# lgleznah/mort

Hardware: AMD Instinct MI355X
Metric: Msamples/sec (width x height x spp/s), Scene 1 1200x675 (higher is better)
Workload: dtype f32; 1 GPU; Scene 1 (random-spheres cover) 1200x675, 500 spp nominal = 484 effective, depth 20, megakernel, seed 69420, host LCG scene; mode=mega, partition=rows/8 interleaved over 1 rank(s)

## Files before the change

mort_amd/csrc/hip/dev_math.h:

```cpp
#ifndef MORT_DEV_MATH_H
#define MORT_DEV_MATH_H

#include <hip/hip_runtime.h>
#include <stdint.h>
#include "mort_math.h"

#pragma clang fp contract(off)

#define DEV __host__ __device__ __forceinline__

struct V3 { float x, y, z; };
DEV V3 mk(float x, float y, float z) { V3 r; r.x = x; r.y = y; r.z = z; return r; }
DEV V3 vadd(V3 a, V3 b) { return mk(a.x + b.x, a.y + b.y, a.z + b.z); }
DEV V3 vsub(V3 a, V3 b) { return mk(a.x - b.x, a.y - b.y, a.z - b.z); }
DEV V3 vmul(V3 a, V3 b) { return mk(a.x * b.x, a.y * b.y, a.z * b.z); }
DEV V3 vneg(V3 a) { return mk(-a.x, -a.y, -a.z); }
DEV V3 vscale(float t, V3 v) { return mk(t * v.x, t * v.y, t * v.z); }
DEV V3 vdiv(V3 v, float t) { return vscale(1 / t, v); }
DEV float vdot(V3 u, V3 v) { return u.x * v.x + u.y * v.y + u.z * v.z; }
DEV float vlen2(V3 a) { return a.x * a.x + a.y * a.y + a.z * a.z; }
DEV float vlen(V3 a) { return mort_sqrtf(vlen2(a)); }
DEV V3 vunit(V3 a) { return vdiv(a, vlen(a)); }
DEV V3 vcross(V3 u, V3 v) { return mk(u.y * v.z - u.z * v.y, u.z * v.x - u.x * v.z, u.x * v.y - u.y * v.x); }

// ... 41 lines not shown
        V3 p = mk(a, b, 0);
        if (vlen2(p) < 1) return p;
    }
}
DEV V3 random_cosine_direction(Rng &s) {
    float r1 = random_float(s);
    float r2 = random_float(s);
    float phi = (float)(2 * 3.1415926 * (double)r1);
    float sq = mort_sqrtf(r2);
    float sn, cs;
    mort_sincosf(phi, &sn, &cs);
    float x = cs * sq;
    float y = sn * sq;
    float z = mort_sqrtf(1 - r2);
    return mk(x, y, z);
}
DEV V3 reflect(V3 v, V3 n) { return vsub(v, vscale(2 * vdot(v, n), n)); }
DEV V3 refract(V3 uv, V3 n, float etai_over_etat) {
    double cos_theta = mort_fmin((double)vdot(vneg(uv), n), 1.0);
    V3 r_out_perp = vscale(etai_over_etat, vadd(uv, vscale((float)cos_theta, n)));
    V3 r_out_parallel = vscale((float)(-mort_sqrt(mort_fabs(1.0 - (double)vlen2(r_out_perp)))), n);
    return vadd(r_out_perp, r_out_parallel);
}
DEV float reflectance(float cosine, float ref_idx) {
    float r0 = (1 - ref_idx) / (1 + ref_idx);
    r0 = r0 * r0;
    return r0 + (1 - r0) * mort_powi5f(1 - cosine);
}

struct Onb { V3 u, v, w; };
DEV Onb onb_from_w(V3 w) {
    Onb o;
    V3 unit_w = vunit(w);
    V3 a = ((double)mort_fabsf(unit_w.x) > 0.9) ? mk(0, 1, 0) : mk(1, 0, 0);
    V3 v = vunit(vcross(unit_w, a));
    V3 u = vcross(unit_w, v);
    o.u = u; o.v = v; o.w = unit_w;
    return o;
}
DEV V3 onb_local(const Onb &o, V3 a) { return vadd(vadd(vscale(a.x, o.u), vscale(a.y, o.v)), vscale(a.z, o.w)); }

#endif
```

mort_amd/csrc/hip/dev_scene.h:

```cpp
#ifndef MORT_DEV_SCENE_H
#define MORT_DEV_SCENE_H

#include <stdint.h>
#include "mort_scene.h"

#define DREF(type, idx) (((uint32_t)(type) << 16) | (uint32_t)(idx))
#define DREF_TYPE(r) ((int)((r) >> 16) & 0x7fff)
#define DREF_IDX(r) ((int)((r) & 0xffffu))

struct __attribute__((aligned(16))) DSphere {
    float cx, cy, cz, radius;
    float vx, vy, vz;
    uint32_t mat;
};

struct __attribute__((aligned(16))) DQuad {
    float Q[3], D;
    float u[3], area;
    float v[3]; uint32_t mat;
    float n[3]; uint32_t pad0;
    float w[3]; uint32_t pad1;
};

struct __attribute__((aligned(16))) DBvhNode {
// ... 3 lines not shown
};

struct __attribute__((aligned(16))) DNode2 {
    float x0min, x0max, y0min, y0max;
    float z0min, z0max, x1min, x1max;
    float y1min, y1max, z1min, z1max;
    uint32_t child0, child1;
    float e0, e1;
};
struct __attribute__((aligned(16))) DNode4 {
    float x[3][4], y[3][4], z[3][4], e[4];
    uint32_t child[4];
};
#define MORT_NODE4_X 0
#define MORT_NODE4_Y 3
#define MORT_NODE4_Z 6
#define MORT_NODE4_E 9
#define MORT_NODE4_CHILD 10
struct __attribute__((aligned(16))) DLeaf2 {
    DSphere a, b;
    float xmin, xmax, ymin, ymax, zmin, zmax;
    uint32_t n;
    uint32_t prims;
    uint32_t pad[4];
};
#define MORT_NODE4_PIECES 11
#define MORT_LEAF2_PIECES 7
#define MORT_OWN4_STACK 24
struct __attribute__((aligned(16))) DNodeQ {
    float ox, oy, oz;
    uint32_t exps;
    uint32_t q0;
    uint32_t q1;
    uint32_t q2;
    uint32_t children;
};
#define GLEAF_FIRST(ref) ((ref) & 0x1fffu)
#define GLEAF_COUNT(ref) ((((ref) >> 13) & 3u) + 1u)
#define MORT_OWN_STACK 16
#define MORT_OWN_MAX_DEPTH 15
#ifndef MORT_GEN_LEAF_MAX
#define MORT_GEN_LEAF_MAX 2
#endif
#define GENT(kind, chain, idx) (((uint32_t)(kind) << 31) | ((uint32_t)(chain) << 24) | (uint32_t)(idx))
#define GENT_QUAD(e) ((e) >> 31)
#define GENT_CHAIN(e) (((e) >> 24) & 0x7fu)
#define GENT_IDX(e) ((e) & 0xffffffu)

enum { XF_TRANSLATE = 0, XF_ROTATE_Y = 1 };
struct __attribute__((aligned(16))) DXform {
    int kind;
    float a, b, c;
};

enum { ITEM_BVH = 0, ITEM_SPHERES = 1, ITEM_QUADS = 2, ITEM_MEDIUM = 3 };
struct __attribute__((aligned(16))) DItem {
    int kind;
    int first, count;
    int chain_first, chain_count;
    uint32_t mat;
    int medium;
    int pad0;
};

struct __attribute__((aligned(16))) DLambert { float r, g, b; uint32_t tex; };
struct __attribute__((aligned(16))) DMetal { float r, g, b, fuzz; };
struct __attribute__((aligned(8))) DDielectric { float ior, inv_ior; };
struct __attribute__((aligned(16))) DSolid { float r, g, b, pad; };
struct __attribute__((aligned(16))) DChecker { float inv_scale; uint32_t even, odd; uint32_t pad; };
struct __attribute__((aligned(16))) DImage { uint32_t offset; int width, height, pad; };

enum { LIGHT_NONE = -1, LIGHT_INVALID = 0, LIGHT_SPHERE = 1, LIGHT_QUAD = 2, LIGHT_LIST = 3 };

struct DScene {
    const DItem *items;     int n_items;
    const DItem *subitems;  int n_subitems;
    const DBvhNode *nodes;  int n_nodes;
    const DSphere *spheres; int n_spheres;
    const DQuad *quads;     int n_quads;
    const DXform *xforms;   int n_xforms;
    const double *neg_inv_density; int n_media;
    const DLambert *lambert; const DMetal *metal; const DDielectric *dielectric;
    const DLambert *dlight;  const DLambert *isotropic;
    const DSolid *solid; const DChecker *checker; const DImage *image;
    const DImage *image_hbm;
    const unsigned char *texels;
    const float *noise;
    const DSphere *wspheres; const DQuad *wquads;
    const int *list_types; const int *list_idxs;
    const int *list_first; const int *list_count;
// ... 6 lines not shown
```

mort_amd/csrc/hip/mega_bvh.h:

```cpp
#ifndef MORT_MEGA_BVH_H
#define MORT_MEGA_BVH_H

#include "dev_render.h"


struct FastArgs {
    RenderArgs r;
    const unsigned char *hot_src;
    uint32_t hot_bytes;
    uint32_t off_nodes4, off_leafrecs, off_lambert, off_metal, off_diel, off_dlight, off_iso, off_solid, off_checker;
    uint32_t off_tstack;
    int node_first, node_count;
    unsigned int *next_q;
    int tiles_x, tiles_total;
    uint32_t off_stack;
    int stack_lds_depth;
    const unsigned *tile_order;
    int gen_tiles;
    int spread_shift;
    unsigned *tile_cost;
    int th_s, th_l, t_keep;
    int sub;
    float *vaccum;
    float4 *deep;
// ... 71 lines not shown
            if (sphere_hit_t(spheres[p], ray, ray_a, 0.001f, closest, t)) { closest = t; best = (int)p; }
        }
        n = skip;
    }
    RefHit h; h.best = best; h.closest = closest;
    return h;
}

DEV float sphere_hit_root(const DSphere &s, const Ray &r, float a, float t_min, float t_max) {
    const V3 oc = vsub(r.o, sphere_center(s, r.tm));
    const float half_b = vdot(oc, r.d);
    const float c = vlen2(oc) - s.radius * s.radius;
    const float discriminant = half_b * half_b - a * c;
    if (discriminant < 0) return -1.0f;
    const float sqrtd = mort_sqrtf(discriminant);
    float root = (-half_b - sqrtd) / a;
    if (root < t_min || t_max < root) {
        root = (-half_b + sqrtd) / a;
        if (root < t_min || t_max < root) return -1.0f;
    }
    return root;
}

struct OwnRay { float ix, iy, iz, mx, my, mz, band, invlen; };

DEV bool own_prune(float xmin, float xmax, float ymin, float ymax, float zmin, float zmax, float e, const OwnRay &r, float closest, float &te_out) {
    const float px0 = __builtin_fmaf(xmin, r.ix, -r.mx), px1 = __builtin_fmaf(xmax, r.ix, -r.mx);
    const float py0 = __builtin_fmaf(ymin, r.iy, -r.my), py1 = __builtin_fmaf(ymax, r.iy, -r.my);
    const float pz0 = __builtin_fmaf(zmin, r.iz, -r.mz), pz1 = __builtin_fmaf(zmax, r.iz, -r.mz);
    const float te = __builtin_fmaxf(__builtin_fmaxf(__builtin_fminf(px0, px1), __builtin_fminf(py0, py1)),
                                     __builtin_fmaxf(__builtin_fminf(pz0, pz1), 0.001f));
    const float tx = __builtin_fminf(__builtin_fminf(__builtin_fmaxf(px0, px1), __builtin_fmaxf(py0, py1)), __builtin_fmaxf(pz0, pz1));
    const float tau = __builtin_fmaf(__builtin_fmaxf(mort_fabsf(te), mort_fabsf(tx)), 9.5367431640625e-07f, r.band);
    const float key = __builtin_fmaf(te, 0.992f, -__builtin_fmaf(e, r.invlen, tau));
    te_out = te;
    return (tx - te < -tau) || (key > closest);
}

DEV bool own_prune_ordered(float xn, float xf, float yn, float yf, float zn, float zf, float e, const OwnRay &r, float closest, float &te_out) {
    const float pxn = __builtin_fmaf(xn, r.ix, -r.mx), pxf = __builtin_fmaf(xf, r.ix, -r.mx);
    const float pyn = __builtin_fmaf(yn, r.iy, -r.my), pyf = __builtin_fmaf(yf, r.iy, -r.my);
    const float pzn = __builtin_fmaf(zn, r.iz, -r.mz), pzf = __builtin_fmaf(zf, r.iz, -r.mz);
    const float te = __builtin_fmaxf(__builtin_fmaxf(pxn, pyn), __builtin_fmaxf(pzn, 0.001f));
    const float tx = __builtin_fminf(__builtin_fminf(pxf, pyf), pzf);
    const float tau = __builtin_fmaf(__builtin_fmaxf(mort_fabsf(te), mort_fabsf(tx)), 9.5367431640625e-07f, r.band);
    const float key = __builtin_fmaf(te, 0.992f, -__builtin_fmaf(e, r.invlen, tau));
    te_out = te;
// ... 214 lines not shown
    {
        const uint32_t *src = (const uint32_t *)fap;
        uint32_t *dst = (uint32_t *)&s_fa;
        for (uint32_t i = threadIdx.x; i < (uint32_t)(sizeof(FastArgs) / 4); i += BLOCK) dst[i] = src[i];
    }
#endif
    {
        const uint4 *src = (const uint4 *)fap->hot_src;
        uint4 *dst = (uint4 *)lds;
        const uint32_t n16 = fap->hot_bytes >> 4;
        for (uint32_t i = threadIdx.x; i < n16; i += BLOCK) dst[i] = src[i];
    }
    __syncthreads();
    if (threadIdx.x == 0) cam_view_fill(s_cam, s_fa.r);
    __syncthreads();
    const FastArgs &L = s_fa;
    static_assert(sizeof(DNode4) == 16 * MORT_NODE4_PIECES && sizeof(DLeaf2) == 16 * MORT_LEAF2_PIECES, "record strides");
    const float4 *nodes4 = (const float4 *)(lds + BU_U(L.off_nodes4));
    const float4 *leafrecs = (const float4 *)(lds + BU_U(L.off_leafrecs));
    unsigned short *const ts_base = (unsigned short *)(lds + BU_U(L.off_tstack)) + threadIdx.x;
#define TS_AT(ptr) (*(ptr))
    const DLambert *lambert = (const DLambert *)(lds + BU_U(L.off_lambert));
    const DMetal *metal = (const DMetal *)(lds + BU_U(L.off_metal));
    const DDielectric *dielectric = (const DDielectric *)(lds + BU_U(L.off_diel));
    const DLambert *dlight = (const DLambert *)(lds + BU_U(L.off_dlight));
    const DLambert *isotropic = (const DLambert *)(lds + BU_U(L.off_iso));
    const DSolid *solid = (const DSolid *)(lds + BU_U(L.off_solid));
    const DChecker *checker = (const DChecker *)(lds + BU_U(L.off_checker));

    const int node_first = BU_I(L.node_first), node_end = node_first + BU_I(L.node_count);
    const int th_s = BU_I(L.th_s), th_l = BU_I(L.th_l), t_keep = BU_I(L.t_keep);
    const int sqrt_spp = BU_I(L.r.sqrt_spp), bounce_limit = BU_I(L.r.bounce_limit);
    const float bg_x = BU_F(L.r.background.x), bg_y = BU_F(L.r.background.y), bg_z = BU_F(L.r.background.z);
    const int spp = sqrt_spp * sqrt_spp;
    const unsigned total_q = (unsigned)BU_I(L.tiles_total) * 64u;

    int state = ((int)(threadIdx.x & 63u) < BU_I(L.lane_cap)) ? ST_S : ST_DONE, kind = K_NEWPIX;
    int xy = 0, lofs = 0;
    Rng rng; rng.d = rng.v0 = rng.v1 = rng.v2 = rng.v3 = rng.v4 = 0; rng.draws = 0;
    V3 pixel_color = mk(0, 0, 0);
    int s_ij = 0, iter = 0;
    uint32_t segments = 0;
    Ray ray; ray.o = mk(0, 0, 0); ray.d = mk(0, 0, 1); ray.tm = 0;
    float ray_time0 = 0;
    OwnRay orr; orr.ix = orr.iy = orr.iz = 1; orr.mx = orr.my = orr.mz = 0; orr.band = 0; orr.invlen = 1;
    float ray_a = 1, closest = 0;
    int best = -1;
// ... 119 lines not shown
                    if (!have) { state = ST_S; kind = K_SHADE; }
                    else { node = next & 0x7fffu; if (next & 0x8000u) state = ST_L; }
                }
                }
                keep = __popcll(__ballot(state == ST_T));
                if (DRAIN && leader >= 0) keep = drain_rounds ? (keep > 0 ? 64 : 0) : (__builtin_amdgcn_readlane(state, leader) == ST_T) ? 64 : 0;
                else if (keep > 0 && keep < t_keep) {
                    const int wL = __popcll(__ballot(state == ST_L)), wS = __popcll(__ballot(state == ST_S));
                    if (!(wS >= e_s || wL >= e_l)) keep = 64;
                }
            } while (keep >= t_keep);
            PROFC(0);
        }
        if (pick == ST_L) {
                REGION("L");
            PROF(1, nL);
            if (state == ST_L) {
                const float4 *lp = leafrecs + node;
                const float4 a0 = lp[0], a1 = lp[1], b0 = lp[2], b1 = lp[3];
                const uint32_t two = ((const uint4 *)lp)[5].z;
                DSphere sa, sb;
                sa.cx = a0.x; sa.cy = a0.y; sa.cz = a0.z; sa.radius = a0.w; sa.vx = a1.x; sa.vy = a1.y; sa.vz = a1.z; sa.mat = __float_as_uint(a1.w);
                sb.cx = b0.x; sb.cy = b0.y; sb.cz = b0.z; sb.radius = b0.w; sb.vx = b1.x; sb.vy = b1.y; sb.vz = b1.z; sb.mat = __float_as_uint(b1.w);
                const float ta = sphere_hit_root(sa, ray, ray_a, 0.001f, closest);
                if (ta != -1.0f) {
                    if (ta == closest && best >= 0) flags |= FL_TIE;
                    closest = ta; best = (int)(node << 16);
                }
                if (two == 2u) {
                    const float tb = sphere_hit_root(sb, ray, ray_a, 0.001f, closest);
                    if (tb != -1.0f) {
                        if (tb == closest && best >= 0) flags |= FL_TIE;
                        closest = tb; best = (int)((node << 16) | 0x8000u);
                    }
                }
                if (spa != ts_base) {
                    spa -= BLOCK;
                    const uint32_t next = TS_AT(spa);
                    node = next & 0x7fffu;
                    state = (next & 0x8000u) ? ST_L : ST_T;
                } else { state = ST_S; kind = K_SHADE; }
            }
            PROFC(1);
        }
      }
      if (!running) break;
        {
            PROF(2, nS);
            PROFS0();
            V3 final_value = mk(0, 0, 0);
                REGION("S:verify");
            if (state == ST_S) {
                if (kind == K_SHADE) {
                    bool need_ref = (flags & FL_MASK) != 0;
                    if (!need_ref && best >= 0) {
                        const float4 *lp = leafrecs + (best >> 16);
                        const float4 b0 = lp[4], b1 = lp[5];
                        DBvhNode lb;
                        lb.xmin = b0.x; lb.xmax = b0.y; lb.ymin = b0.z; lb.ymax = b0.w; lb.zmin = b1.x; lb.zmax = b1.y; lb.skip = 0; lb.prims = 0;
                        need_ref = !slab_check(lb, ray, orr, closest);
                    }
                    if (need_ref) {
                        atomicAdd(&fap->r.counters[3], 1ull);
                        const RefHit h = reference_walk(fap->r.sc.nodes, node_first, node_end, fap->r.sc.spheres, ray.o.x, ray.o.y, ray.o.z,
                                                        ray.d.x, ray.d.y, ray.d.z, ray.tm, ray_a);
                        best = h.best; closest = h.closest;
                    }
                    PROFF(0);
                REGION("S:hitrecord");
                    if (best < 0) {
                        final_value = mk(bg_x, bg_y, bg_z);
                        kind = K_FINISH;
                    } else {
                        DSphere sp;
                        if (need_ref) sp = fap->r.sc.spheres[best];
                        else {
                            const float4 *lp = leafrecs + (best >> 16) + ((best & 0x8000) ? 2 : 0);
                            const float4 s0 = lp[0], s1 = lp[1];
                            sp.cx = s0.x; sp.cy = s0.y; sp.cz = s0.z; sp.radius = s0.w; sp.vx = s1.x; sp.vy = s1.y; sp.vz = s1.z; sp.mat = __float_as_uint(s1.w);
                        }
                        const V3 p = ray_at(ray, closest);
                        const V3 outward = vdiv(vsub(p, sphere_center(sp, ray.tm)), sp.radius);
                        const bool front_face = vdot(ray.d, outward) < 0;
                        const V3 normal = front_face ? outward : vneg(outward);
                        const int mtype = DREF_TYPE(sp.mat), midx = DREF_IDX(sp.mat);
                        PROFF(1);
                        StackEntry e;
                        if (mtype == MORT_MAT_METAL) {
                REGION("S:metal");
                            PROFB(0);
                            const DMetal m = metal[midx];
                            V3 reflected = reflect(ray.d, normal);
                            reflected = vadd(vunit(reflected), vscale(m.fuzz, random_unit_vector(rng)));
                            ray.o = p; ray.d = reflected;
                            e.kx = 1.0f * m.r; e.ky = 1.0f * m.g; e.kz = 1.0f * m.b; e.rp = 1.0f;
                            PROFF(2);
                        } else if (mtype == MORT_MAT_DIELECTRIC) {
                REGION("S:dielectric");
                            PROFB(1);
                            const DDielectric m = dielectric[midx];
                            const float refraction_ratio = front_face ? m.inv_ior : m.ior;
                            const V3 unit_direction = vunit(ray.d);
                            const float cos_theta = (float)mort_fmin((double)vdot(vneg(unit_direction), normal), 1.0);
                            const float sin_theta = (float)mort_sqrt(1.0 - (double)(cos_theta * cos_theta));
                            const bool cant_refract = (double)(refraction_ratio * sin_theta) > 1.0;
                            V3 direction;
                            if (cant_refract || reflectance(cos_theta, refraction_ratio) > random_float(rng))
                                direction = reflect(unit_direction, normal);
                            else
                                direction = refract(unit_direction, normal, refraction_ratio);
                            ray.o = p; ray.d = direction;
                            e.kx = 1.0f; e.ky = 1.0f; e.kz = 1.0f; e.rp = 1.0f;
                            ident_mask |= (1ull << iter);
                            PROFF(3);
                        } else if (mtype == MORT_MAT_LAMBERTIAN || mtype == MORT_MAT_ISOTROPIC) {
                REGION("S:lambertian");
                            PROFB(2);
                            const bool lamb = (mtype == MORT_MAT_LAMBERTIAN);
                            const DLambert m = lamb ? lambert[midx] : isotropic[midx];
                            V3 attenuation = mk(m.r, m.g, m.b);
                            if (m.tex != 0) {
                                uint32_t tex = m.tex;
                                bool resolved = false;
                                for (int guard = 0; guard < 8 && !resolved; guard++) {
                                    const int tt = DREF_TYPE(tex), ti = DREF_IDX(tex);
                                    if (tt == MORT_TEXTURE_SOLID) { const DSolid sc = solid[ti]; attenuation = mk(sc.r, sc.g, sc.b); resolved = true; }
                                    else if (tt == MORT_TEXTURE_CHECKER) {
                                        const DChecker c = checker[ti];
                                        const int xi = mort_f2i(mort_floorf(c.inv_scale * p.x));
                                        const int yi = mort_f2i(mort_floorf(c.inv_scale * p.y));
// ... 101 lines not shown
                        if (spp <= 0) {
                            final_value = mk(0, 0, 0);
                        }
                    }
                }
                REGION("S:getray");
                PROFS(6);
                if (state != ST_DONE) {
                    if (kind == K_NEWSAMPLE) {
                        PROFB(4);
                        ray = get_ray(s_cam, xy & 0xffff, (xy >> 16) & 0x7fff, rng, s_ij & 0xffff, s_ij >> 16);
                        ray_time0 = ray.tm;
                        iter = 0;
                        kind = K_SHADE;
                        if (bounce_limit <= 0) { final_value = mk(0, 0, 0); kind = K_FINISH; }
                    }
                REGION("S:setup");
                    if (kind == K_SHADE) {
                        ray_a = vlen2(ray.d);
                        orr.ix = 1.0f / ray.d.x; orr.iy = 1.0f / ray.d.y; orr.iz = 1.0f / ray.d.z;
                        orr.mx = ray.o.x * orr.ix; orr.my = ray.o.y * orr.iy; orr.mz = ray.o.z * orr.iz;
                        const float mm = __builtin_fmaxf(__builtin_fmaxf(mort_fabsf(orr.mx), mort_fabsf(orr.my)), mort_fabsf(orr.mz));
                        orr.band = mm * 4.76837158203125e-07f;
                        orr.invlen = 1.01f / mort_sqrtf(ray_a);
                        const bool ordinary = own_inv_ok(orr.ix) && own_inv_ok(orr.iy) && own_inv_ok(orr.iz) && (mm < 1e30f);
                        closest = __builtin_inff();
                        best = -1;
                        node = 0; spa = ts_base;
                        flags = ordinary ? FL_SIGNS(own_sign_offset(orr.ix), own_sign_offset(orr.iy), own_sign_offset(orr.iz)) : FL_REF;
                        segments++;
                        state = ordinary ? ST_T : ST_S;
                    }
                }
            }
                REGION("S:end");
            if (DRAIN && __ballot(state == ST_DONE) != 0ull) {
                unsigned key = (state <= ST_S) ? ((unsigned)((s_ij >> 16) * sqrt_spp + (s_ij & 0xffff)) << 6) | (threadIdx.x & 63u) : 0xffffffffu;
                for (int off = 32; off > 0; off >>= 1) { const unsigned o = (unsigned)__shfl_xor((int)key, off); key = o < key ? o : key; }
                leader = (key == 0xffffffffu) ? -1 : __builtin_amdgcn_readfirstlane((int)(key & 63u));
            }
            PROFS(7);
            PROFC(2);
        }
    }
    if ((threadIdx.x & 63) == 0) {
#ifdef MORT_PROFILE_STATES
#ifdef MORT_PROFILE_FINE
        for (int k = 0; k < 12; k++) atomicAdd(&counters_p[18 + k], proff[k]);
// ... 17 lines not shown
```

mort_amd/csrc/hip/mort_hip.hip:

```cpp
#include <hip/hip_runtime.h>

#include <algorithm>
#include <array>
#include <climits>
#include <cmath>
#include <cstdio>
#include <cstdlib>
#include <cstring>
#include <new>
#include <string>
#include <thread>
#include <vector>

#include "mort_hip.h"
#include "dev_pixel.h"
#include "scene_blob.h"
#include "seed_host.h"
#include "mort_internal.h"
#include "mort_ctx.h"
#include "mega_gen.h"
#include "wave_gen.h"

#pragma clang fp contract(off)

// ... 193 lines not shown
    c->have_world = c->fast_ok = c->gen_ok = c->wave_ok = false;
    if (c->d_fast) { hipFree(c->d_fast); c->d_fast = nullptr; }
    if (c->d_trav) { hipFree(c->d_trav); c->d_trav = nullptr; }
    if (c->d_gen) { hipFree(c->d_gen); c->d_gen = nullptr; }
    int st;
    SceneBlob sb;
    st = build_scene_blob(w, sb);
    if (st != MORT_OK) return st;
    const mortc::Compiled &o = sb.comp;
    void *d = nullptr;
    HIPCHK(c, hipMalloc(&d, sb.bytes.size()));
    hipError_t e = hipMemcpy(d, sb.bytes.data(), sb.bytes.size(), hipMemcpyHostToDevice);
    if (e != hipSuccess) { hipFree(d); return hip_fail(c, e, "hipMemcpy(scene)"); }
    if (c->d_scene) hipFree(c->d_scene);
    c->d_scene = d;
    scene_view(sb, (const unsigned char *)d, c->sc);
    c->list_types = o.list_types; c->list_idxs = o.list_idxs;
    for (int i = 0; i < MORT_NUM_HITTABLE_LIST; i++) { c->list_first[i] = o.list_first[i]; c->list_count[i] = o.list_count[i]; }
    c->n_wspheres = (int)o.wspheres.size(); c->n_wquads = (int)o.wquads.size(); c->n_lists = w->objs.num_hittable_list;
    c->wave_ok = (o.items.size() == 1 && o.items[0].kind == ITEM_BVH && o.quads.empty());
    if (c->wave_ok && !o.own_nodes.empty() && !o.own_nodes4.empty()) {
        std::vector<unsigned char> fb, tb;
        c->f_nodes4 = (uint32_t)place(fb, o.own_nodes4); c->f_leafrecs = (uint32_t)place(fb, o.own_leafrecs);
        c->f_lambert = (uint32_t)place(fb, o.lambert); c->f_metal = (uint32_t)place(fb, o.metal); c->f_diel = (uint32_t)place(fb, o.dielectric);
        c->f_dlight = (uint32_t)place(fb, o.dlight); c->f_iso = (uint32_t)place(fb, o.isotropic);
        c->f_solid = (uint32_t)place(fb, o.solid); c->f_checker = (uint32_t)place(fb, o.checker);
        fb.resize((fb.size() + 15) & ~(size_t)15, 0);
        c->t_nodes2 = (uint32_t)place(tb, o.own_nodes); c->t_leaves = (uint32_t)place(tb, o.own_leaves); c->t_spheres = (uint32_t)place(tb, o.spheres);
        tb.resize((tb.size() + 15) & ~(size_t)15, 0);
        if (fb.size() <= 72 * 1024 && tb.size() <= 72 * 1024) {
            HIPCHK(c, hipMalloc(&c->d_fast, fb.size()));
            HIPCHK(c, hipMemcpy(c->d_fast, fb.data(), fb.size(), hipMemcpyHostToDevice));
            HIPCHK(c, hipMalloc(&c->d_trav, tb.size()));
            HIPCHK(c, hipMemcpy(c->d_trav, tb.data(), tb.size(), hipMemcpyHostToDevice));
            c->fast_bytes = (uint32_t)fb.size(); c->trav_bytes = (uint32_t)tb.size();
            c->own_nodes = (int)o.own_nodes.size(); c->own_leaves = (int)o.own_leaves.size(); c->own4_stack = o.own4_stack > 1 ? o.own4_stack : 1;
            c->fast_ok = true;
        }
    }
    if (o.g_ok && !std::getenv("MORT_NO_GEN")) {
        std::vector<unsigned char> gb;
        GenArgs g;
        std::memset(&g, 0, sizeof g);
        g.o_nodes = (uint32_t)place(gb, o.g_nodes); g.o_leaves = g.o_nodes; g.o_entries = (uint32_t)place(gb, o.g_entries);
        g.o_chains = (uint32_t)place(gb, o.g_chains); g.o_xforms = (uint32_t)place(gb, o.xforms);
        g.o_items = (uint32_t)place(gb, o.items); g.o_subitems = (uint32_t)place(gb, o.subitems); g.o_media = (uint32_t)place(gb, o.media);
        g.o_lambert = (uint32_t)place(gb, o.lambert); g.o_metal = (uint32_t)place(gb, o.metal); g.o_diel = (uint32_t)place(gb, o.dielectric);
// ... 705 lines not shown
            for (size_t ni = r % (size_t)stride; ni < nodes.size(); ni += (size_t)stride) {
                const DNode4 &nd = nodes[ni];
                for (int k = 0; k < 4; k++) {
                    if (nd.child[k] == 0xffffu) continue;
                    float te_a, te_b;
                    const bool skip_a = own_prune(nd.x[0][k], nd.x[1][k], nd.y[0][k], nd.y[1][k], nd.z[0][k], nd.z[1][k], nd.e[k], orr, closest, te_a);
                    const bool skip_b = own_prune_ordered(nd.x[sx][k], nd.x[sx + 1][k], nd.y[sy][k], nd.y[sy + 1][k], nd.z[sz][k], nd.z[sz + 1][k], nd.e[k], orr, closest, te_b);
                    o[0]++;
                    if (std::memcmp(&te_a, &te_b, 4) != 0) o[1]++;
                    if (skip_a != skip_b) o[2]++;
                    if (skip_a && skip_b) o[6]++;
                }
            }
        }
    };
    std::vector<std::thread> pool;
    for (unsigned t = 1; t < nthreads; t++) pool.emplace_back(work, t);
    work(0);
    for (std::thread &th : pool) th.join();
    for (const auto &o : part) for (int i = 0; i < 16; i++) if (i != 4 && i != 5) out[i] += o[i];
    return MORT_OK;
}

extern "C" int mort_hip_render_device(mort_ctx *c, const mort_camera *cam, int mode, void *d_rgba, void *d_accum,
                                      void *stream, mort_stats *stats) {
    return render_device_impl(c, cam, mode, d_rgba, d_accum, nullptr, stream, stats);
}

extern "C" int mort_hip_render(mort_ctx *c, const mort_camera *cam, int mode, uint8_t *rgba_out, float *accum_out,
                               uint32_t *segments_px_out, mort_stats *stats) {
    if (!c || !cam || !rgba_out) return MORT_ERR_INVALID;
    const int W = cam->image_width, H = cam->image_height;
    if (W <= 0 || H <= 0) return MORT_ERR_INVALID;
    HIPCHK(c, hipSetDevice(c->device));
    const int lr = local_rows_for(c->part, H);
    const size_t npx = (size_t)W * (size_t)lr;
    int st;
    if ((st = ensure_buf(c, &c->d_rgba, &c->rgba_cap, npx * 4)) != MORT_OK) return st;
    if (accum_out && (st = ensure_buf(c, &c->d_accum, &c->accum_cap, npx * 12)) != MORT_OK) return st;
    if (segments_px_out) { if ((st = ensure_buf(c, &c->d_segpx, &c->segpx_cap, npx * 4)) != MORT_OK) return st; }
    else if (c->d_segpx) { hipFree(c->d_segpx); c->d_segpx = nullptr; c->segpx_cap = 0; }
    mort_stats local;
    st = render_device_impl(c, cam, mode, c->d_rgba, accum_out ? c->d_accum : nullptr,
                            segments_px_out ? (uint32_t *)c->d_segpx : nullptr, nullptr, &local);
    if (st != MORT_OK) return st;
    if (stats) *stats = local;
// ... 15 lines not shown
```

mort_amd/csrc/hip/scene_compile.h:

```cpp
#ifndef MORT_SCENE_COMPILE_H
#define MORT_SCENE_COMPILE_H

#include <algorithm>
#include <cmath>
#include <cstdlib>
#include <cstring>
#include <vector>

#include "dev_scene.h"
#include "mort_hip.h"

namespace mortc {

static const int kMaxChain = 8;
static const int kMaxDepth = 16;

struct Ref { int kind; int idx; int cf, cc; };

struct Compiled {
    std::vector<DItem> items, subitems;
    std::vector<DBvhNode> nodes;
    std::vector<DSphere> spheres, wspheres;
    std::vector<DQuad> quads, wquads;
    std::vector<DXform> xforms;
    std::vector<double> media;
    std::vector<DLambert> lambert, dlight, isotropic;
    std::vector<DMetal> metal;
    std::vector<DDielectric> dielectric;
    std::vector<DSolid> solid;
    std::vector<DChecker> checker;
    std::vector<DImage> image;
    std::vector<unsigned char> texels;
    std::vector<unsigned char> noise;
    std::vector<int> list_types, list_idxs;
    int list_first[MORT_NUM_HITTABLE_LIST], list_count[MORT_NUM_HITTABLE_LIST];
    int status = MORT_OK;
    bool inverted_box = false;
    std::vector<DNode2> own_nodes;
    std::vector<DBvhNode> own_leaves;
    int own_depth = 0;
    std::vector<DLeaf2> own_leafrecs;
    std::vector<DNode4> own_nodes4;
    int own4_stack = 0;
    bool g_ok = false;
    std::vector<DNodeQ> g_nodes;
    std::vector<uint32_t> g_entries;
    std::vector<int> g_chains;
    std::vector<uint32_t> g_ranks;
    uint32_t g_root = 0xffffu;
    int g_first_medium = 0;
    int g_depth = 0;
// ... 240 lines not shown
            if ((nd.prims & 0x8000u) || ((nd.prims >> 16) & 0x8000u)) return;
            Box b;
            b.lo[0] = nd.xmin; b.hi[0] = nd.xmax; b.lo[1] = nd.ymin; b.hi[1] = nd.ymax; b.lo[2] = nd.zmin; b.hi[2] = nd.zmax;
            for (int k = 0; k < 3; k++) if (!std::isfinite(b.lo[k]) || !std::isfinite(b.hi[k]) || b.lo[k] > b.hi[k]) return;
            ob.lb.push_back(b); ob.ldiag.push_back(box_diag(b));
            leaves.push_back(nd);
        }
        const int n = (int)leaves.size();
        if (n < 2 || n > 0x7fff) return;
        std::vector<int> ids(n);
        for (int i = 0; i < n; i++) ids[i] = i;
        Box rb; float re;
        const uint32_t root = own_emit(ob, ids, 0, n, 0, rb, re);
        if (root != 0 || out.own_nodes.size() > 0x7fff || ob.max_depth_seen + 1 > MORT_OWN_MAX_DEPTH) { out.own_nodes.clear(); return; }
        for (const DNode2 &nd : out.own_nodes) if (!std::isfinite(nd.e0) || !std::isfinite(nd.e1)) { out.own_nodes.clear(); return; }
        out.own_leaves = leaves;
        out.own_depth = ob.max_depth_seen + 1;
        for (const DBvhNode &lf : leaves) {
            DLeaf2 r;
            std::memset(&r, 0, sizeof r);
            const uint32_t pa = lf.prims & 0x7fffu, pb = (lf.prims >> 16) & 0x7fffu;
            if (pa >= out.spheres.size() || pb >= out.spheres.size()) { out.own_nodes.clear(); out.own_leaves.clear(); return; }
            r.a = out.spheres[pa]; r.b = out.spheres[pb]; r.n = pa == pb ? 1u : 2u; r.prims = pa | (pb << 16);
            r.xmin = lf.xmin; r.xmax = lf.xmax; r.ymin = lf.ymin; r.ymax = lf.ymax; r.zmin = lf.zmin; r.zmax = lf.zmax;
            out.own_leafrecs.push_back(r);
        }
        collapse_own_tree();
    }
    struct Slot4 { uint32_t ref; float lo[3], hi[3], e; };
    static Slot4 slot_of(const DNode2 &nd, int k) {
        Slot4 s;
        s.ref = k ? nd.child1 : nd.child0; s.e = k ? nd.e1 : nd.e0;
        s.lo[0] = k ? nd.x1min : nd.x0min; s.hi[0] = k ? nd.x1max : nd.x0max;
        s.lo[1] = k ? nd.y1min : nd.y0min; s.hi[1] = k ? nd.y1max : nd.y0max;
        s.lo[2] = k ? nd.z1min : nd.z0min; s.hi[2] = k ? nd.z1max : nd.z0max;
        return s;
    }
    struct Cut4 { double t[5]; unsigned char left[5]; };
    void cut_expand(const std::vector<Cut4> &dp, const Slot4 &s, int k, std::vector<Slot4> &outv) const {
        if ((s.ref & 0x8000u) || dp[s.ref].left[k] == 0) { outv.push_back(s); return; }
        const int i = dp[s.ref].left[k];
        cut_expand(dp, slot_of(out.own_nodes[s.ref], 0), i, outv);
        cut_expand(dp, slot_of(out.own_nodes[s.ref], 1), k - i, outv);
    }
    int collapse_emit(const std::vector<Cut4> &dp, uint32_t b2, uint32_t me) {
        std::vector<Slot4> sl;
// ... 357 lines not shown
            for (int i = 0; i < o.num_constant_medium; i++) if (!o.host_constant_medium[i].skip) refs.push_back({3, i, 0, 0});
            for (int i = 0; i < o.num_hittable_list; i++) if (!o.host_hittable_list[i].skip) flatten(MORT_OBJ_HITTABLE_LIST, i, 0, 0, 0, refs);
            emit_items(refs, out.items, true);
        }
        build_own_tree();
        build_unified();
        for (int i = 0; i < o.num_spheres; i++) out.wspheres.push_back(to_dsphere(o.host_sphere[i]));
        for (int i = 0; i < o.num_quads; i++) out.wquads.push_back(to_dquad(o.host_quad[i]));
        for (int i = 0; i < MORT_NUM_HITTABLE_LIST; i++) { out.list_first[i] = 0; out.list_count[i] = 0; }
        for (int i = 0; i < o.num_hittable_list && i < MORT_NUM_HITTABLE_LIST; i++) {
            const mort_hittable_list &l = o.host_hittable_list[i];
            out.list_first[i] = (int)out.list_types.size();
            out.list_count[i] = l.num_objs;
            for (int k = 0; k < l.num_objs; k++) { out.list_types.push_back(l.obj_types[k]); out.list_idxs.push_back(l.obj_idxs[k]); }
        }
        const mort_world_materials &m = w->mats;
        for (int i = 0; i < m.num_lambertians; i++) out.lambert.push_back(tex_material(m.host_lambertian[i].texType, m.host_lambertian[i].texIdx));
        for (int i = 0; i < m.num_diffuse_lights; i++) out.dlight.push_back(tex_material(m.host_diffuse_light[i].texType, m.host_diffuse_light[i].texIdx));
        for (int i = 0; i < m.num_isotropics; i++) out.isotropic.push_back(tex_material(m.host_isotropic[i].texType, m.host_isotropic[i].texIdx));
        for (int i = 0; i < m.num_metals; i++) {
            DMetal d; d.r = m.host_metal[i].albedo.e[0]; d.g = m.host_metal[i].albedo.e[1]; d.b = m.host_metal[i].albedo.e[2]; d.fuzz = m.host_metal[i].fuzz;
            out.metal.push_back(d);
        }
        for (int i = 0; i < m.num_dielectrics; i++) { DDielectric d; d.ior = m.host_dielectric[i].ior; d.inv_ior = m.host_dielectric[i].inv_ior; out.dielectric.push_back(d); }
        const mort_world_textures &t = w->texs;
        for (int i = 0; i < t.num_solid_colors; i++) {
            DSolid d; d.r = t.host_solid_color[i].color_value.e[0]; d.g = t.host_solid_color[i].color_value.e[1]; d.b = t.host_solid_color[i].color_value.e[2]; d.pad = 0;
            out.solid.push_back(d);
        }
        for (int i = 0; i < t.num_checker_textures; i++) {
            const mort_checker_texture &c = t.host_checker_texture[i];
            DChecker d; d.inv_scale = c.inv_scale; d.even = tex_ref(c.evenTextureType, c.evenTextureIdx); d.odd = tex_ref(c.oddTextureType, c.oddTextureIdx); d.pad = 0;
            out.checker.push_back(d);
        }
        for (int i = 0; i < t.num_image_textures; i++) {
            const mort_image_texture &im = t.host_image_texture[i];
            DImage d; d.offset = (uint32_t)out.texels.size(); d.width = im.texels ? im.width : 0; d.height = im.texels ? im.height : 0; d.pad = 0;
            if (im.texels && im.width > 0 && im.height > 0)
                out.texels.insert(out.texels.end(), im.texels, im.texels + (size_t)im.width * im.height * 3);
            out.image.push_back(d);
        }
        for (int i = 0; i < t.num_noise_textures; i++) {
            const unsigned char *p = (const unsigned char *)&t.host_noise_texture[i];
            out.noise.insert(out.noise.end(), p, p + sizeof(mort_noise_texture));
        }
    }
};
// ... 5 lines not shown
```

Measured before the change: 4226 Msamples/s.

## Replace divisions with precomputed reciprocals and refined rcp in sphere leaf tests

Tests both leaf spheres together and replaces the IEEE divisions in the quadratic roots with one hardware reciprocal per ray plus Newton-refined quotients. Rays whose magnitudes could break that refinement fall back to the reference path. The per-sphere inverse radius and per-dielectric Schlick r0 terms are precomputed on the host into spare padding and a widened material struct, removing a division from each normal computation and from each reflectance call. The inverse ray length now uses rsq, and a debug kernel checks that the short division agrees with full division. The cost is extra bounds checks and a branch, plus the risk of tiny rounding differences versus the reference.

```diff
diff --git a/mort_amd/csrc/hip/dev_math.h b/mort_amd/csrc/hip/dev_math.h
--- a/mort_amd/csrc/hip/dev_math.h
+++ b/mort_amd/csrc/hip/dev_math.h
@@ -87,11 +87,12 @@
     V3 r_out_parallel = vscale((float)(-mort_sqrt(mort_fabs(1.0 - (double)vlen2(r_out_perp)))), n);
     return vadd(r_out_perp, r_out_parallel);
 }
-DEV float reflectance(float cosine, float ref_idx) {
+DEV float schlick_r0(float ref_idx) {
     float r0 = (1 - ref_idx) / (1 + ref_idx);
-    r0 = r0 * r0;
-    return r0 + (1 - r0) * mort_powi5f(1 - cosine);
+    return r0 * r0;
 }
+DEV float reflectance_r0(float cosine, float r0) { return r0 + (1 - r0) * mort_powi5f(1 - cosine); }
+DEV float reflectance(float cosine, float ref_idx) { return reflectance_r0(cosine, schlick_r0(ref_idx)); }
 
 struct Onb { V3 u, v, w; };
 DEV Onb onb_from_w(V3 w) {
diff --git a/mort_amd/csrc/hip/dev_scene.h b/mort_amd/csrc/hip/dev_scene.h
--- a/mort_amd/csrc/hip/dev_scene.h
+++ b/mort_amd/csrc/hip/dev_scene.h
@@ -49,7 +49,8 @@
     float xmin, xmax, ymin, ymax, zmin, zmax;
     uint32_t n;
     uint32_t prims;
-    uint32_t pad[4];
+    float inv_ra, inv_rb;
+    uint32_t pad[2];
 };
 #define MORT_NODE4_PIECES 11
 #define MORT_LEAF2_PIECES 7
@@ -93,6 +94,7 @@
 struct __attribute__((aligned(16))) DLambert { float r, g, b; uint32_t tex; };
 struct __attribute__((aligned(16))) DMetal { float r, g, b, fuzz; };
 struct __attribute__((aligned(8))) DDielectric { float ior, inv_ior; };
+struct __attribute__((aligned(16))) DDielectricR0 { float ior, inv_ior, r0_front, r0_back; };
 struct __attribute__((aligned(16))) DSolid { float r, g, b, pad; };
 struct __attribute__((aligned(16))) DChecker { float inv_scale; uint32_t even, odd; uint32_t pad; };
 struct __attribute__((aligned(16))) DImage { uint32_t offset; int width, height, pad; };
diff --git a/mort_amd/csrc/hip/mega_bvh.h b/mort_amd/csrc/hip/mega_bvh.h
--- a/mort_amd/csrc/hip/mega_bvh.h
+++ b/mort_amd/csrc/hip/mega_bvh.h
@@ -117,7 +117,51 @@
     return root;
 }
 
+#define MORT_SHORT_DIV_A_MIN 9.094947017729282e-13f
+#define MORT_SHORT_DIV_A_MAX 1099511627776.0f
+#define MORT_SHORT_DIV_X_MAX 1073741824.0f
+DEV bool short_div_a_ok(float a) { return a > MORT_SHORT_DIV_A_MIN && a < MORT_SHORT_DIV_A_MAX; }
+DEV bool short_div_x_ok(float half_b, float disc) { return mort_fabsf(half_b) < MORT_SHORT_DIV_X_MAX && disc < MORT_SHORT_DIV_X_MAX * MORT_SHORT_DIV_X_MAX; }
+DEV float short_div_rcp(float a) {
+#if defined(__HIP_DEVICE_COMPILE__)
+    const float r = __builtin_amdgcn_rcpf(a);
+    return __builtin_fmaf(__builtin_fmaf(-a, r, 1.0f), r, r);
+#else
+    (void)a; return 0.0f;
+#endif
+}
+DEV float short_div(float x, float a, float r) {
+#if defined(__HIP_DEVICE_COMPILE__)
+    float q = x * r;
+    float e = __builtin_fmaf(-a, q, x);
+    q = __builtin_fmaf(e, r, q);
+    e = __builtin_fmaf(-a, q, x);
+    return __builtin_fmaf(e, r, q);
+#else
+    (void)r; return x / a;
+#endif
+}
+DEV void sphere_hit_terms(const DSphere &s, const Ray &r, float a, float &half_b, float &discriminant) {
+    const V3 oc = vsub(r.o, sphere_center(s, r.tm));
+    half_b = vdot(oc, r.d);
+    const float c = vlen2(oc) - s.radius * s.radius;
+    discriminant = half_b * half_b - a * c;
+}
+DEV bool sphere_hit_pick(bool in, float q_near, float q_far, float t_min, float t_max, float &root) {
+    const bool near_out = q_near < t_min || t_max < q_near;
+    const bool far_out = q_far < t_min || t_max < q_far;
+    root = near_out ? q_far : q_near;
+    return in && !(near_out && far_out);
+}
+
 struct OwnRay { float ix, iy, iz, mx, my, mz, band, invlen; };
+DEV float own_invlen(float ray_a) {
+#if defined(__HIP_DEVICE_COMPILE__)
+    return 1.01f * __builtin_amdgcn_rsqf(ray_a);
+#else
+    return 1.01f / mort_sqrtf(ray_a);
+#endif
+}
 
 DEV bool own_prune(float xmin, float xmax, float ymin, float ymax, float zmin, float zmax, float e, const OwnRay &r, float closest, float &te_out) {
     const float px0 = __builtin_fmaf(xmin, r.ix, -r.mx), px1 = __builtin_fmaf(xmax, r.ix, -r.mx);
@@ -378,7 +422,7 @@
 #define TS_AT(ptr) (*(ptr))
     const DLambert *lambert = (const DLambert *)(lds + BU_U(L.off_lambert));
     const DMetal *metal = (const DMetal *)(lds + BU_U(L.off_metal));
-    const DDielectric *dielectric = (const DDielectric *)(lds + BU_U(L.off_diel));
+    const DDielectricR0 *dielectric = (const DDielectricR0 *)(lds + BU_U(L.off_diel));
     const DLambert *dlight = (const DLambert *)(lds + BU_U(L.off_dlight));
     const DLambert *isotropic = (const DLambert *)(lds + BU_U(L.off_iso));
     const DSolid *solid = (const DSolid *)(lds + BU_U(L.off_solid));
@@ -544,16 +588,26 @@
                 DSphere sa, sb;
                 sa.cx = a0.x; sa.cy = a0.y; sa.cz = a0.z; sa.radius = a0.w; sa.vx = a1.x; sa.vy = a1.y; sa.vz = a1.z; sa.mat = __float_as_uint(a1.w);
                 sb.cx = b0.x; sb.cy = b0.y; sb.cz = b0.z; sb.radius = b0.w; sb.vx = b1.x; sb.vy = b1.y; sb.vz = b1.z; sb.mat = __float_as_uint(b1.w);
-                const float ta = sphere_hit_root(sa, ray, ray_a, 0.001f, closest);
-                if (ta != -1.0f) {
-                    if (ta == closest && best >= 0) flags |= FL_TIE;
-                    closest = ta; best = (int)(node << 16);
-                }
-                if (two == 2u) {
-                    const float tb = sphere_hit_root(sb, ray, ray_a, 0.001f, closest);
-                    if (tb != -1.0f) {
-                        if (tb == closest && best >= 0) flags |= FL_TIE;
-                        closest = tb; best = (int)((node << 16) | 0x8000u);
+                float hba, da, hbb, db;
+                sphere_hit_terms(sa, ray, ray_a, hba, da);
+                sphere_hit_terms(sb, ray, ray_a, hbb, db);
+                const bool in_a = !(da < 0), in_b = two == 2u && !(db < 0);
+                if (in_a || in_b) {
+                    if (!(short_div_x_ok(hba, da) && short_div_x_ok(hbb, db))) flags |= FL_REF;
+                    else {
+                        const float sqa = mort_sqrtf(da), sqb = mort_sqrtf(db);
+                        const float rcp_a = short_div_rcp(ray_a);
+                        const float qa0 = short_div(-hba - sqa, ray_a, rcp_a), qa1 = short_div(-hba + sqa, ray_a, rcp_a);
+                        const float qb0 = short_div(-hbb - sqb, ray_a, rcp_a), qb1 = short_div(-hbb + sqb, ray_a, rcp_a);
+                        float ta, tb;
+                        if (sphere_hit_pick(in_a, qa0, qa1, 0.001f, closest, ta)) {
+                            if (ta == closest && best >= 0) flags |= FL_TIE;
+                            closest = ta; best = (int)(node << 16);
+                        }
+                        if (sphere_hit_pick(in_b, qb0, qb1, 0.001f, closest, tb)) {
+                            if (tb == closest && best >= 0) flags |= FL_TIE;
+                            closest = tb; best = (int)((node << 16) | 0x8000u);
+                        }
                     }
                 }
                 if (spa != ts_base) {
@@ -595,14 +649,16 @@
                         kind = K_FINISH;
                     } else {
                         DSphere sp;
-                        if (need_ref) sp = fap->r.sc.spheres[best];
+                        float inv_radius;
+                        if (need_ref) { sp = fap->r.sc.spheres[best]; inv_radius = 1 / sp.radius; }
                         else {
                             const float4 *lp = leafrecs + (best >> 16) + ((best & 0x8000) ? 2 : 0);
                             const float4 s0 = lp[0], s1 = lp[1];
                             sp.cx = s0.x; sp.cy = s0.y; sp.cz = s0.z; sp.radius = s0.w; sp.vx = s1.x; sp.vy = s1.y; sp.vz = s1.z; sp.mat = __float_as_uint(s1.w);
+                            inv_radius = ((const float *)(leafrecs + (best >> 16) + 6))[(best & 0x8000) ? 1 : 0];
                         }
                         const V3 p = ray_at(ray, closest);
-                        const V3 outward = vdiv(vsub(p, sphere_center(sp, ray.tm)), sp.radius);
+                        const V3 outward = vscale(inv_radius, vsub(p, sphere_center(sp, ray.tm)));
                         const bool front_face = vdot(ray.d, outward) < 0;
                         const V3 normal = front_face ? outward : vneg(outward);
                         const int mtype = DREF_TYPE(sp.mat), midx = DREF_IDX(sp.mat);
@@ -620,14 +676,15 @@
                         } else if (mtype == MORT_MAT_DIELECTRIC) {
                 REGION("S:dielectric");
                             PROFB(1);
-                            const DDielectric m = dielectric[midx];
+                            const DDielectricR0 m = dielectric[midx];
                             const float refraction_ratio = front_face ? m.inv_ior : m.ior;
+                            const float r0 = front_face ? m.r0_front : m.r0_back;
                             const V3 unit_direction = vunit(ray.d);
                             const float cos_theta = (float)mort_fmin((double)vdot(vneg(unit_direction), normal), 1.0);
                             const float sin_theta = (float)mort_sqrt(1.0 - (double)(cos_theta * cos_theta));
                             const bool cant_refract = (double)(refraction_ratio * sin_theta) > 1.0;
                             V3 direction;
-                            if (cant_refract || reflectance(cos_theta, refraction_ratio) > random_float(rng))
+                            if (cant_refract || reflectance_r0(cos_theta, r0) > random_float(rng))
                                 direction = reflect(unit_direction, normal);
                             else
                                 direction = refract(unit_direction, normal, refraction_ratio);
@@ -775,8 +832,8 @@
                         orr.mx = ray.o.x * orr.ix; orr.my = ray.o.y * orr.iy; orr.mz = ray.o.z * orr.iz;
                         const float mm = __builtin_fmaxf(__builtin_fmaxf(mort_fabsf(orr.mx), mort_fabsf(orr.my)), mort_fabsf(orr.mz));
                         orr.band = mm * 4.76837158203125e-07f;
-                        orr.invlen = 1.01f / mort_sqrtf(ray_a);
-                        const bool ordinary = own_inv_ok(orr.ix) && own_inv_ok(orr.iy) && own_inv_ok(orr.iz) && (mm < 1e30f);
+                        orr.invlen = own_invlen(ray_a);
+                        const bool ordinary = own_inv_ok(orr.ix) && own_inv_ok(orr.iy) && own_inv_ok(orr.iz) && (mm < 1e30f) && short_div_a_ok(ray_a);
                         closest = __builtin_inff();
                         best = -1;
                         node = 0; spa = ts_base;
diff --git a/mort_amd/csrc/hip/mort_hip.hip b/mort_amd/csrc/hip/mort_hip.hip
--- a/mort_amd/csrc/hip/mort_hip.hip
+++ b/mort_amd/csrc/hip/mort_hip.hip
@@ -239,7 +239,7 @@
     if (c->wave_ok && !o.own_nodes.empty() && !o.own_nodes4.empty()) {
         std::vector<unsigned char> fb, tb;
         c->f_nodes4 = (uint32_t)place(fb, o.own_nodes4); c->f_leafrecs = (uint32_t)place(fb, o.own_leafrecs);
-        c->f_lambert = (uint32_t)place(fb, o.lambert); c->f_metal = (uint32_t)place(fb, o.metal); c->f_diel = (uint32_t)place(fb, o.dielectric);
+        c->f_lambert = (uint32_t)place(fb, o.lambert); c->f_metal = (uint32_t)place(fb, o.metal); c->f_diel = (uint32_t)place(fb, o.dielectric_r0);
         c->f_dlight = (uint32_t)place(fb, o.dlight); c->f_iso = (uint32_t)place(fb, o.isotropic);
         c->f_solid = (uint32_t)place(fb, o.solid); c->f_checker = (uint32_t)place(fb, o.checker);
         fb.resize((fb.size() + 15) & ~(size_t)15, 0);
@@ -991,6 +991,57 @@
     return MORT_OK;
 }
 
+__global__ void __launch_bounds__(256) short_div_check_kernel(const float *a_vals, const float *q_vals, uint32_t nq, unsigned long long *out) {
+    __shared__ unsigned long long s_cnt[4];
+    if (threadIdx.x < 4) s_cnt[threadIdx.x] = 0ull;
+    __syncthreads();
+    const float a = a_vals[blockIdx.x];
+    const bool a_ok = short_div_a_ok(a);
+    const float r = short_div_rcp(a);
+    unsigned long long cnt[4] = {0ull, 0ull, 0ull, 0ull};
+    for (uint32_t j = threadIdx.x; j < nq; j += 256u) {
+        const float q = q_vals[j];
+        const uint32_t pb = __float_as_uint(a * q);
+        for (int k = 0; k < 6; k++) {
+            const float x = k == 0 ? q : __uint_as_float(pb + (uint32_t)(k - 3));
+            if (!(a_ok && mort_fabsf(x) < 2.0f * MORT_SHORT_DIV_X_MAX)) { cnt[2]++; continue; }
+            cnt[0]++;
+            const float full = x / a;
+            const float sh = short_div(x, a, r);
+            if (__float_as_uint(full) == __float_as_uint(sh)) continue;
+            bool same = (full < 9.5367431640625e-07f) && ((full < 0.001f) == (sh < 0.001f));
+            const float cl[3] = {0.001f, 1.0f, __builtin_inff()};
+            for (int c = 0; c < 3; c++) same = same && ((full < 0.001f || cl[c] < full) == (sh < 0.001f || cl[c] < sh));
+            if (same) { cnt[3]++; continue; }
+            cnt[1]++;
+            if (atomicCAS(&out[4], 0ull, 1ull) == 0ull) {
+                out[5] = __float_as_uint(a); out[6] = __float_as_uint(x); out[7] = __float_as_uint(full); out[8] = __float_as_uint(sh);
+            }
+        }
+    }
+    for (int i = 0; i < 4; i++) if (cnt[i]) atomicAdd(&s_cnt[i], cnt[i]);
+    __syncthreads();
+    if (threadIdx.x < 4 && s_cnt[threadIdx.x]) atomicAdd(&out[threadIdx.x], s_cnt[threadIdx.x]);
+}
+extern "C" int mort_hip_debug_short_forms(int device, const float *a_vals, size_t na, const float *q_vals, size_t nq, unsigned long long *out) {
+    if (!a_vals || !q_vals || !out || na < 1 || nq < 1 || na > (1u << 20) || nq > (1u << 20)) return MORT_ERR_INVALID;
+    if (hipSetDevice(device) != hipSuccess) return MORT_ERR_HIP;
+    float *d_a = nullptr, *d_q = nullptr;
+    unsigned long long *d_out = nullptr;
+    bool ok = hipMalloc(&d_a, na * sizeof(float)) == hipSuccess && hipMalloc(&d_q, nq * sizeof(float)) == hipSuccess &&
+              hipMalloc(&d_out, 16 * sizeof(unsigned long long)) == hipSuccess;
+    ok = ok && hipMemcpy(d_a, a_vals, na * sizeof(float), hipMemcpyHostToDevice) == hipSuccess &&
+         hipMemcpy(d_q, q_vals, nq * sizeof(float), hipMemcpyHostToDevice) == hipSuccess &&
+         hipMemset(d_out, 0, 16 * sizeof(unsigned long long)) == hipSuccess;
+    if (ok) {
+        hipLaunchKernelGGL(short_div_check_kernel, dim3((unsigned)na), dim3(256), 0, 0, d_a, d_q, (uint32_t)nq, d_out);
+        ok = hipGetLastError() == hipSuccess && hipDeviceSynchronize() == hipSuccess &&
+             hipMemcpy(out, d_out, 16 * sizeof(unsigned long long), hipMemcpyDeviceToHost) == hipSuccess;
+    }
+    hipFree(d_a); hipFree(d_q); hipFree(d_out);
+    return ok ? MORT_OK : MORT_ERR_HIP;
+}
+
 extern "C" int mort_hip_render_device(mort_ctx *c, const mort_camera *cam, int mode, void *d_rgba, void *d_accum,
                                       void *stream, mort_stats *stats) {
     return render_device_impl(c, cam, mode, d_rgba, d_accum, nullptr, stream, stats);
diff --git a/mort_amd/csrc/hip/scene_compile.h b/mort_amd/csrc/hip/scene_compile.h
--- a/mort_amd/csrc/hip/scene_compile.h
+++ b/mort_amd/csrc/hip/scene_compile.h
@@ -8,6 +8,7 @@
 #include <vector>
 
 #include "dev_scene.h"
+#include "dev_math.h"
 #include "mort_hip.h"
 
 namespace mortc {
@@ -27,6 +28,7 @@
     std::vector<DLambert> lambert, dlight, isotropic;
     std::vector<DMetal> metal;
     std::vector<DDielectric> dielectric;
+    std::vector<DDielectricR0> dielectric_r0;
     std::vector<DSolid> solid;
     std::vector<DChecker> checker;
     std::vector<DImage> image;
@@ -313,6 +315,7 @@
             const uint32_t pa = lf.prims & 0x7fffu, pb = (lf.prims >> 16) & 0x7fffu;
             if (pa >= out.spheres.size() || pb >= out.spheres.size()) { out.own_nodes.clear(); out.own_leaves.clear(); return; }
             r.a = out.spheres[pa]; r.b = out.spheres[pb]; r.n = pa == pb ? 1u : 2u; r.prims = pa | (pb << 16);
+            r.inv_ra = 1.0f / r.a.radius; r.inv_rb = 1.0f / r.b.radius;
             r.xmin = lf.xmin; r.xmax = lf.xmax; r.ymin = lf.ymin; r.ymax = lf.ymax; r.zmin = lf.zmin; r.zmax = lf.zmax;
             out.own_leafrecs.push_back(r);
         }
@@ -716,7 +719,8 @@
             DMetal d; d.r = m.host_metal[i].albedo.e[0]; d.g = m.host_metal[i].albedo.e[1]; d.b = m.host_metal[i].albedo.e[2]; d.fuzz = m.host_metal[i].fuzz;
             out.metal.push_back(d);
         }
-        for (int i = 0; i < m.num_dielectrics; i++) { DDielectric d; d.ior = m.host_dielectric[i].ior; d.inv_ior = m.host_dielectric[i].inv_ior; out.dielectric.push_back(d); }
+        for (int i = 0; i < m.num_dielectrics; i++) { DDielectric d; d.ior = m.host_dielectric[i].ior; d.inv_ior = m.host_dielectric[i].inv_ior; out.dielectric.push_back(d);
+            DDielectricR0 r; r.ior = d.ior; r.inv_ior = d.inv_ior; r.r0_front = schlick_r0(d.inv_ior); r.r0_back = schlick_r0(d.ior); out.dielectric_r0.push_back(r); }
         const mort_world_textures &t = w->texs;
         for (int i = 0; i < t.num_solid_colors; i++) {
             DSolid d; d.r = t.host_solid_color[i].color_value.e[0]; d.g = t.host_solid_color[i].color_value.e[1]; d.b = t.host_solid_color[i].color_value.e[2]; d.pad = 0;
```

Result: faster. 4310 Msamples/s (median of 6 runs) (+2.0%).
